# noisystreet/aither

Hardware: AMD Instinct MI355X
Metric: Mcell-updates/sec per iteration (residual+LU-SGS), 256^3 block; % HBM roofline (higher is better)
Workload: dtype f64

## Files before the change

aither_amd/csrc/agx_api.hip:

```cpp
#include "agx_kernels.hpp"
#include "agx_geometry.hpp"
#include "agx_mem.hpp"
#include <rccl/rccl.h>
#include <cstdarg>
#include <cstdio>
#include <cstring>
#include <cstdlib>
#include <cmath>
#include <vector>
#include <array>
#include <map>
#include <string>
#include <algorithm>

using namespace agx;

static char g_err[512] = "";
static int fail(const char* fmt, ...) {
  va_list ap;
  va_start(ap, fmt);
  vsnprintf(g_err, sizeof g_err, fmt, ap);
  va_end(ap);
  return 1;
}
// ... 25 lines not shown
    for (auto& g1 : g) for (auto& g2 : g1) for (auto& g3 : g2)
      if (g3) { hipGraphExecDestroy(g3); g3 = nullptr; }
  }
};

struct Block {
  BlockDev d;
  int global_pos = 0;
  DevBuf<double> slab;
  DevBuf<double> d2;
  DevBuf<double> blockmat;
  DevBuf<double> sweep_rec;
  bool sweep_geo_built = false;
  bool x_planes_current = false;
  bool x_is_zero = false;
  DevBuf<double> mg_forcing, mg_mres, mg_xsave, mg_nodes;
  DevBuf<int> mg_tc, mg_start;
  DevBuf<double> mg_vf, mg_cf;
  const void *mg_tc_key = nullptr, *mg_vf_key = nullptr, *mg_cf_key = nullptr;
  bool node_built = false;
  DevBuf<double> nodes_dev, fcen;
  DevBuf<int> d2_tab;
  std::vector<int> dstart;
  SweepGraphs sweep_graph;
  DevBuf<int> kp_mem;
  unsigned kp_epoch = 0;
  long d2idx(int i, int j, int k) const {
    const int ie = i + d.ng, je = j + d.ng, de = ie + je;
    return (long)(k + d.ng) * d.d2.ps + dstart[de] + je - std::max(0, de - (d.d2.Pi - 1));
  }
// ... 97 lines not shown
  bool halo_batch_required = false;
  int halo_batch_sides = 0;
  long halo_batch_nmax = 0;
  std::vector<int> halo_conn_order;
  struct HaloLevel { int first, sides; long nmax; };
  std::vector<HaloLevel> halo_levels;
  DevBuf<HaloSide> halo_tab_dev[5][2][2];
  bool halo_tab_valid[5][2] = {};
  int halo_set[5] = {};
  PinnedBuf<HaloSide> halo_tab_host;
  int tile_order_inv = TILE_ORDER_STEP;
  int tile_order_visc = TILE_ORDER_STEP;
  std::map<std::array<int, 6>, TilePlan> tile_plans;
  int mresid_split = 1;
  bool mresid_march = true;
  bool have_time_n = false;
  bool have_wall_data = false;
  bool in_iterate = false, ghosts_prefilled = false;
  bool ghost_fill_open = false;
  bool mres_deferred = false;
  hipEvent_t norm_event = nullptr;
  bool consn_pending = false;
  bool state_is_time_n = false;
  long fused_parts = 0;
  bool timing = false;
  std::vector<std::pair<hipEvent_t, hipEvent_t>> ev_pool;
  std::vector<std::pair<int, int>> ev_used;
  double t_ms[G_NGROUP] = {};
  long t_n[G_NGROUP] = {};
};
// ... 84 lines not shown
    HIPCHK(c->stage_buf.alloc(doubles));
  }
  *out = c->stage_buf.get();
  return 0;
}
static int copy_out(agx_ctx* c, double* out, const double* dev, size_t n) {
  HIPCHK(hipGetLastError());
  HIPCHK(hipMemcpyAsync(out, dev, sizeof(double) * n, hipMemcpyDeviceToHost, c->stream));
  HIPCHK(hipStreamSynchronize(c->stream));
  return 0;
}
int upload_aos(agx_ctx* c, Block& b, const double* host, double* const* dst,
               int ncomp, int ci, int cj, int ck, int gsrc) {
  const long n = (long)ci * cj * ck;
  double* tmp = nullptr;
  if (stage_buffer(c, (size_t)n * ncomp, &tmp)) return 1;
  HIPCHK(hipMemcpyAsync(tmp, host, sizeof(double) * n * ncomp,
                        hipMemcpyHostToDevice, c->stream));
  hipLaunchKernelGGL(k_aos_to_soa, dim3((n + 255) / 256), dim3(256), 0,
                     c->stream, tmp, planes(dst, ncomp), ncomp, ci, cj, ck, gsrc, b.d);
  HIPCHK(hipGetLastError());
  HIPCHK(hipStreamSynchronize(c->stream));
  return 0;
}
int download_aos(agx_ctx* c, Block& b, double* host, double* const* src,
                 int ncomp, int ci, int cj, int ck, int gsrc) {
  const long n = (long)ci * cj * ck;
  double* tmp = nullptr;
  if (stage_buffer(c, (size_t)n * ncomp, &tmp)) return 1;
  hipLaunchKernelGGL(k_soa_to_aos, dim3((n + 255) / 256), dim3(256), 0,
// ... 64 lines not shown
      }
}

int ensure_halo_buf(agx_ctx* c, long ndoubles) {
  bool grew;
  HIPCHK(c->halo_buf.reserve((size_t)ndoubles, &grew));
  if (grew)
    for (auto& v : c->halo_tab_valid) v[0] = v[1] = false;
  return 0;
}

int halo_in_d2(const Block& b, int what) { return what == AGX_HALO_UPDATE && b.d.d2.base ? 1 : 0; }
void x_changed(agx_ctx* c) {
  for (auto& blk : c->blocks) blk.x_planes_current = false;
}
Planes5 halo_planes(Block& b, int what) {
  Planes5 r;
  r.rec = what == AGX_HALO_UPDATE ? b.d.sw_dyn : nullptr;
  const bool z2 = halo_in_d2(b, what) != 0;
  r.stride = z2 ? 2 : 1;
#if AGX_NEQ == 7
  if (what == AGX_HALO_TURB) {
    for (int e = 0; e < AGX_NEQ; ++e) r.p[e] = b.d.turb3[e < 3 ? e : 2];
    return r;
  }
#endif
  if (what == AGX_HALO_VELGRAD_A || what == AGX_HALO_VELGRAD_B) {
    for (int e = 0; e < AGX_NEQ; ++e) {
      const int comp = what == AGX_HALO_VELGRAD_A ? e : std::min(5 + e, 8);
      r.p[e] = b.d.vg + (long)comp * b.d.nplane;
// ... 553 lines not shown
  HIPCHK(hipGetLastError());
  return 0;
}

int bc_faces(agx_ctx* c) { Timer t(c, G_BC); return bc_pass(c, true, 0); }
int bc_edges(agx_ctx* c) { Timer t(c, G_BC); return bc_pass(c, false, 0); }

int fill_ghosts(agx_ctx* c) {
  if (bc_faces(c)) return 1;
  if (agx_halo_exchange(c, AGX_HALO_STATE)) return 1;
  return bc_edges(c);
}
int update_pass(agx_ctx* c, int mode, int mm, double* l2, agx_linf* linf) {
  c->state_is_time_n = false;
  const double alpha[4] = {0.25, 1.0 / 3.0, 0.5, 1.0};
  if (mode != 2 && c->fused_pending) {
    Timer t(c, G_UPDATE);
    long off = 0;
    for (size_t n = 0; n < c->blocks.size(); ++n) {
      BlockDev& b = c->blocks[n].d;
      const MarchPlan mp = march_plan(c, b);
      hipLaunchKernelGGL(k_norm_final, dim3(1), dim3(256), 0, c->stream,
                         c->partials.get() + off, mp.nparts, c->norm_out.get() + n);
      off += mp.nparts;
      for (int e = 0; e < AGX_NEQ; ++e) std::swap(b.state[e], b.state2[e]);
    }
    c->halo_set[AGX_HALO_STATE] ^= 1;
    c->fused_pending = false;
    HIPCHK(hipGetLastError());
  } else {
    Timer t(c, G_UPDATE);
    for (size_t n = 0; n < c->blocks.size(); ++n) {
      const BlockDev& b = c->blocks[n].d;
      const int last = mm == c->cfg.nonlinear_iterations - 1;
#if AGX_FAST
      if (mode == 2 && b.d2.base) {
        const dim3 tg((b.ni + TT - 1) / TT, (b.nj + TT - 1) / TT, b.nk);
        hipLaunchKernelGGL(k_update_d2, tg, dim3(256), 0, c->stream, b, c->gas, c->sp, last,
                           c->partials.get());
        if (reduce_norms(c, n, (long)tg.x * tg.y * tg.z)) return 1;
        continue;
      }
#endif
      const dim3 grid = cell_grid(b, CELL_BLOCK);
      hipLaunchKernelGGL(k_update, grid, CELL_BLOCK, 0, c->stream, b, c->gas,
                         c->sp, mode, mode == 1 ? alpha[mm & 3] : 1.0, last,
                         c->partials.get());
      if (reduce_norms(c, n, (long)grid.x * grid.y * grid.z)) return 1;
    }
  }
  HIPCHK(hipMemcpyAsync(c->norm_host.get(), c->norm_out.get(),
                        sizeof(NormPartial) * c->blocks.size(),
                        hipMemcpyDeviceToHost, c->stream));
  if (c->mres_deferred)
    HIPCHK(hipMemcpyAsync(c->norm_host.get() + c->blocks.size(),
                          c->norm_out.get() + c->blocks.size() + 64,
                          sizeof(NormPartial) * c->blocks.size(), hipMemcpyDeviceToHost,
                          c->stream));
  HIPCHK(hipMemcpyAsync(c->err_host.get(), c->err_dev.get(), sizeof(int),
                        hipMemcpyDeviceToHost, c->stream));
  if (c->in_iterate && c->eager_ghosts) {
    if (!c->norm_event) HIPCHK(hipEventCreateWithFlags(&c->norm_event, hipEventDisableTiming));
    HIPCHK(hipEventRecord(c->norm_event, c->stream));
    if (fill_ghosts(c)) return 1;
    c->ghosts_prefilled = true;
    HIPCHK(hipEventSynchronize(c->norm_event));
// ... 393 lines not shown
        return fail("AGX_TILE_ORDER is '%s': step or column", w);
      }
      c->tile_order_inv = c->tile_order_visc = !strcmp(w, "step") ? TILE_ORDER_STEP : TILE_ORDER_COLUMN;
    }
    if (const char* w = getenv("AGX_EAGER_GHOSTS")) c->eager_ghosts = atoi(w) != 0;
    if (const char* w = getenv("AGX_OVERLAP")) c->overlap = atoi(w) != 0;
    if (const char* w = getenv("AGX_LUSGS")) c->lusgs_mode = !strcmp(w, "plane") ? 0 : 1;
    if (const char* w = getenv("AGX_SPIN_LIMIT")) c->spin_limit = std::max(1, atoi(w));
    if (const char* w = getenv("AGX_GRAPHS")) c->use_graphs = atoi(w) != 0;
    if (const char* w = getenv("AGX_SWEEP_ALL")) c->sweep_all_launch = atoi(w) != 0;
    if (const char* w = getenv("AGX_SWEEP_PIPE")) c->sweep_pipe = atoi(w) != 0;
    if (const char* w = getenv("AGX_SWEEP_THREE")) c->sweep_three = atoi(w) != 0;
    if (const char* w = getenv("AGX_SWEEP_RECORDS")) c->sweep_records = atoi(w) != 0;
    if (const char* w = getenv("AGX_MRESID_SPLIT")) c->mresid_split = std::min(64, std::max(1, atoi(w)));
    if (const char* w = getenv("AGX_MRESID")) c->mresid_march = strcmp(w, "plane") != 0;
    if (const char* w = getenv("AGX_HALO_BATCH")) {
      c->halo_batch = strcmp(w, "0") != 0;
      c->halo_batch_required = !strcmp(w, "require");
    }
  }
  HIPCHK(c->err_dev.alloc(1));
  HIPCHK(hipMemset(c->err_dev.get(), 0, sizeof(int)));
  HIPCHK(c->err_host.alloc(1));
  *c->err_host.get() = 0;
  *out = c;
  return 0;
}

void agx_ctx_destroy(agx_ctx* c) {
  if (!c) return;
// ... 541 lines not shown
  }
  return 0;
}
}

int agx_setup_finalize(agx_ctx* c) {
  HIPCHK(hipSetDevice(c->device));
  const int ng = c->cfg.n_ghost;
  if (!c->blocks.empty() && c->blocks[0].node_built && geo_complete(c)) return 1;
  long max_parts = 1, max_halo = 1;
  long march_parts = 0;
  for (auto& blk : c->blocks) {
    const dim3 g = cell_grid(blk.d, CELL_BLOCK);
    max_parts = std::max(max_parts, (long)g.x * g.y * g.z);
    march_parts += march_plan(c, blk.d).nparts;
    if (blk.d.d2.base)
      max_parts = std::max(max_parts, mresid_wgs(c, blk.d));
  }
  max_parts = std::max(max_parts, march_parts);
  for (auto& k : c->conns) {
    const agx_connection& cc = k.c;
    const bool l0 = cc.rank[0] == c->rank, l1 = cc.rank[1] == c->rank;
    if (!l0 && !l1) continue;
    for (int s = 0; s < 2; ++s) {
      const bool mine = s == 0 ? l0 : l1, partner_mine = s == 0 ? l1 : l0;
      if (!mine) continue;
      const int lb = cc.local_block[s];
      if (lb < 0 || lb >= (int)c->blocks.size()) return fail("connection refers to unknown block");
      const Block* partner = partner_mine ? &c->blocks[cc.local_block[1 - s]] : nullptr;
      for (int space = 0; space < (use_d2(c) ? 2 : 1); ++space)
        if (halo_maps(k, s, space, ng, CellIndex{&c->blocks[lb], space},
                      CellIndex{partner, space}, partner_mine, &max_halo))
// ... 26 lines not shown
    if (!seen) per_peer.emplace_back(sl.peer, 1);
    sl.count = r.count;
    sl.send = hb ? r.hsend.get() : r.send.get();
    sl.recv = hb ? r.hrecv.get() : r.recv.get();
    c->slabs.push_back(sl);
    c->remote.push_back(std::move(r));
  }
  if (c->have_ex) {
    const size_t nrec = 1 + (size_t)c->ex.nranks;
    HIPCHK(c->rec_dev.alloc(nrec));
    HIPCHK(c->rec_host.alloc(nrec));
  }
  c->n_partials = max_parts;
  HIPCHK(c->partials.alloc((size_t)max_parts));
  const size_t nb = std::max<size_t>(c->blocks.size(), 1);
  HIPCHK(c->norm_out.alloc(2 * nb + 64));
  HIPCHK(c->norm_host.alloc(2 * nb));
  c->finalized = true;
  return 0;
}

int agx_state_upload(agx_ctx* c, int id, const double* state) {
  c->ghosts_prefilled = false;
  c->state_is_time_n = false;
  if (flush_consn(c)) return 1;
  if (id < 0 || id >= (int)c->blocks.size()) return fail("bad block id %d", id);
  Block& b = c->blocks[id];
  const BlockDev& d = b.d;
  if (upload_aos(c, b, state, d.state, AGX_NEQ, d.ni + 2 * d.ng,
                 d.nj + 2 * d.ng, d.nk + 2 * d.ng, d.ng))
    return 1;
// ... 354 lines not shown
  if (field >= AGX_FIELD_VOLUME && field <= AGX_FIELD_WALL_DIST)
    return fail("field %d (geometry) cannot be uploaded: it is set when the block is created",
                field);
  if (field_info(b, field, &p, &nc, &gh)) return fail("field %d cannot be uploaded", field);
  const int g = gh ? b.d.ng : 0;
  if (upload_aos(c, b, in, p, nc, b.d.ni + 2 * g, b.d.nj + 2 * g, b.d.nk + 2 * g, g)) return 1;
  if (field == AGX_FIELD_UPDATE) b.x_is_zero = false;
  if (field == AGX_FIELD_UPDATE && b.d.d2.base) return d2_x_copy(c, b, 1);
  return 0;
}

static int implicit_begin(agx_ctx* c, int write_x);
int agx_phase_matrix_residual(agx_ctx* c, double* mr);
static int d2_x_copy(agx_ctx* c, Block& b, int to_d2);
#if AGX_FAST
static void d2_prepare(agx_ctx* c, Block& blk, int write_x, int again);
#endif
namespace {
int mg_solver_ok(agx_ctx* c) {
  if (!c->sp.implicit) return fail("multigrid: implicit time integration only");
  return 0;
}
int mg_x_to_planes(agx_ctx* c, Block& b) {
  return b.d.d2.base && !b.x_planes_current ? d2_x_copy(c, b, 0) : 0;
}
int mg_x_from_planes(agx_ctx* c, Block& b) { return b.d.d2.base ? d2_x_copy(c, b, 1) : 0; }
void mg_x_records(agx_ctx* c, Block& b) {
  if (b.d.sw_dyn)
    hipLaunchKernelGGL(k_mg_x_records, dim3((unsigned)((b.d.nplane + 255) / 256)), dim3(256), 0,
                       c->stream, b.d);
}
// ... 64 lines not shown
  return 0;
}
int mg_order(agx_ctx* producer, agx_ctx* consumer) {
  if (producer->stream != consumer->stream) HIPCHK(hipStreamSynchronize(producer->stream));
  return 0;
}
}

int agx_mg_restrict(agx_ctx* f, agx_ctx* cz, int blk, int what, const int32_t* tc,
                    const double* vf) {
  if (mg_check(f, cz, blk)) return 1;
  Block &bf = f->blocks[blk], &bc = cz->blocks[blk];
  if (what < AGX_MG_STATE || what > AGX_MG_FORCING) return fail("mg_restrict: bad selector %d", what);
  if (what != AGX_MG_FORCING && !vf) return fail("mg_restrict: volume weights missing");
  if (flush_consn(f) || flush_consn(cz)) return 1;
  MgMap m;
  if (mg_maps(f, bf, tc, vf, nullptr, bc.d.ni, bc.d.nj, bc.d.nk, &m)) return 1;
  if (what == AGX_MG_UPDATE && mg_x_to_planes(f, bf)) return 1;
  if (what == AGX_MG_FORCING && mg_x_to_planes(cz, bc)) return 1;
  if (mg_order(f, cz)) return 1;
  if (what == AGX_MG_STATE) {
    for (int e = 0; e < AGX_NEQ; ++e)
      HIPCHK(hipMemsetAsync(bc.d.state[e], 0, sizeof(double) * bc.d.nplane, cz->stream));
    cz->ghosts_prefilled = false;
    cz->state_is_time_n = false;
    cz->mg_coarse = true;
  } else if (what == AGX_MG_UPDATE) {
    for (int e = 0; e < AGX_NEQ; ++e)
      HIPCHK(hipMemsetAsync(bc.d.x[e], 0, sizeof(double) * bc.d.nplane, cz->stream));
  } else {
    if (!bf.d.mg_mres) return fail("mg_restrict: the fine level has no matrix residual yet");
    if (mg_planes(cz, bc, bc.mg_forcing, &bc.d.mg_forcing)) return 1;
  }
  hipLaunchKernelGGL(k_mg_restrict, cell_grid(bc.d, CELL_BLOCK), CELL_BLOCK, 0, cz->stream, bf.d,
                     bc.d, m, what);
  if (what == AGX_MG_FORCING)
    hipLaunchKernelGGL(k_mg_axmb, cell_grid(bc.d, CELL_BLOCK), CELL_BLOCK, 0, cz->stream, bc.d,
                       cz->gas, cz->sp);
  if (what == AGX_MG_UPDATE) {
    mg_x_records(cz, bc);
    if (mg_x_from_planes(cz, bc)) return 1;
  }
#if AGX_FAST
  if (what == AGX_MG_FORCING && bc.d.d2.base) d2_prepare(cz, bc, 0, 1);
#endif
  HIPCHK(hipGetLastError());
  return 0;
}

int agx_mg_matrix_residual(agx_ctx* c, double* mr) {
  if (mg_solver_ok(c)) return 1;
  for (auto& blk : c->blocks) {
    if (mg_planes(c, blk, blk.mg_mres, &blk.d.mg_mres)) return 1;
    if (mg_x_to_planes(c, blk)) return 1;
  }
  c->mres_plane_form = true;
  const int rc = agx_phase_matrix_residual(c, mr);
  c->mres_plane_form = false;
  return rc;
// ... 68 lines not shown
}

int agx_phase_bc_faces(agx_ctx* c) {
  if (bc_faces(c)) return 1;
  c->ghost_fill_open = true;
  return 0;
}
int agx_phase_bc_edges(agx_ctx* c) { return bc_edges(c); }

int agx_phase_residual(agx_ctx* c, int mm, double cfl) {
  if (c->cfg.dt_nondim <= 0.0 && cfl <= 0.0)
    return fail("Neither dt or cfl was specified!");
  c->ghost_fill_open = false;
  c->sp.diag_add = c->mg_coarse ? 1 : 0;
  const bool fuse = can_fuse(c);
  const int store_consn = !c->use_gather && all_tile_ok(c) && c->consn_pending && mm == 0;
  if (store_consn) c->consn_pending = false;
  else if (flush_consn(c)) return 1;
  {
    Timer t(c, G_RESID);
    long off = 0;
    for (auto& blk : c->blocks) {
      const MarchPlan mp = march_plan(c, blk.d);
      MarchArgs ma;
      memset(&ma, 0, sizeof ma);
      ma.kchunk = mp.kchunk;
      ma.mode = c->cfg.time_integration == AGX_TIME_RK4 ? 1 : 0;
      ma.store_consn = store_consn;
      const double rk_alpha[4] = {0.25, 1.0 / 3.0, 0.5, 1.0};
      ma.alpha = rk_alpha[mm & 3];
// ... 101 lines not shown
      Timer t(c, G_BC);
      hipLaunchKernelGGL(k_nr_grads, dim3((blk.nr_max + 255) / 256, blk.d.nsurf), dim3(256), 0,
                         c->stream, blk.d, c->gas);
      HIPCHK(hipGetLastError());
    }
  return 0;
}

int agx_phase_explicit_update(agx_ctx* c, int mm, double* l2, agx_linf* linf) {
  const int mode = c->cfg.time_integration == AGX_TIME_RK4 ? 1 : 0;
  return update_pass(c, mode, mm, l2, linf);
}

static int implicit_begin(agx_ctx* c, int write_x);
#if AGX_FAST
static void d2_prepare(agx_ctx* c, Block& blk, int write_x, int again) {
  const BlockDev& b = blk.d;
  const dim3 grid((b.d2.Pi + TT - 1) / TT, (b.d2.Pj + TT - 1) / TT, b.nk + 2 * b.ng);
  hipLaunchKernelGGL(k_lusgs_prepare, grid, dim3(256), 0, c->stream, b, c->gas, c->sp,
                     write_x, write_x ? (unsigned)(++blk.kp_epoch) & 3u : 0u, again);
}
#endif
int agx_phase_implicit_begin(agx_ctx* c) { return implicit_begin(c, 1); }
static int implicit_begin(agx_ctx* c, int write_x) {
  x_changed(c);
  Timer t(c, G_PREPARE);
  c->sp.un_is_u = c->state_is_time_n ? 1 : 0;
  for (auto& blk : c->blocks) {
    const BlockDev& b = blk.d;
#if AGX_FAST
    if (b.d2.base) {
      bool conn = false;
      for (int q = 0; q < 6; ++q) conn = conn || b.side_conn[q] != 0;
      const int wx = write_x && (c->sp.requires_init || conn) ? 1 : 0;
      d2_prepare(c, blk, wx, 0);
      blk.x_is_zero = write_x && !wx;
      continue;
    }
#endif
    if (!c->sp.requires_init && write_x)
      hipLaunchKernelGGL(k_zero5, dim3((b.nplane + 255) / 256), dim3(256), 0,
                         c->stream, planes(b.x), b.nplane);
    hipLaunchKernelGGL(k_implicit_begin, cell_grid(b, CELL_BLOCK), CELL_BLOCK, 0,
                       c->stream, b, c->gas, c->sp, c->err_dev.get(), write_x);
    if (b.sw_geo) {
      hipLaunchKernelGGL(k_sweep_records, dim3((unsigned)((b.nplane + 255) / 256)), dim3(256), 0,
                         c->stream, b, c->sp, blk.sweep_geo_built ? 0 : 1);
      blk.sweep_geo_built = true;
    }
  }
// ... 451 lines not shown
```

aither_amd/csrc/agx_kernels.hpp:

```cpp
#pragma once
#include "agx_device.hpp"
#include "agx_lusgs.hpp"
#include "agx_tile_plan.hpp"

namespace agx {

struct BlockDev {
  int ni, nj, nk, ng;
  int ioff;
  long sx, sxy, nplane;
  int parent;
  double* state[AGX_NEQ];
  double* state2[AGX_NEQ];
  double* fa[3][4];
  double* vol;
  double* cen[3];
  double* wid[3];
  double* resid[AGX_NEQ];
  double* specrad;
  double* dt;
  double* consn[AGX_NEQ];
  double* consnm1[AGX_NEQ];
  double* x[AGX_NEQ];
  double* xold[AGX_NEQ];
// ... 2034 lines not shown
}
__global__ void k_halo_scatter_all(const HaloSide* __restrict__ tab) {
  halo_scatter_side(tab[blockIdx.y], (long)blockIdx.x * blockDim.x + threadIdx.x);
}
__global__ void k_halo_gather(Planes5 a, const long* __restrict__ src, long n,
                              double* __restrict__ buf) {
  halo_gather_side(HaloSide{a, src, n, buf}, (long)blockIdx.x * blockDim.x + threadIdx.x);
}
__global__ void k_halo_scatter(Planes5 a, const long* __restrict__ dst, long n,
                               const double* __restrict__ buf) {
  halo_scatter_side(HaloSide{a, dst, n, const_cast<double*>(buf)},
                    (long)blockIdx.x * blockDim.x + threadIdx.x);
}


__device__ __forceinline__ void norm_block_fold(double* v, double vmax, long long lin,
                                                NormPartial* out) {
  __shared__ double sh[AGX_NEQ + 1][16];
  __shared__ long long shl[16];
  for (int off = 32; off > 0; off >>= 1) {
#pragma unroll
    for (int e = 0; e < AGX_NEQ; ++e) v[e] += __shfl_down(v[e], off, 64);
    const double ov = __shfl_down(vmax, off, 64);
    const long long ol = __shfl_down(lin, off, 64);
    if (ov > vmax || (ov == vmax && ol < lin)) { vmax = ov; lin = ol; }
  }
  const int tid = threadIdx.y * blockDim.x + threadIdx.x;
  const int wave = tid >> 6, lane = tid & 63;
  if (lane == 0) {
#pragma unroll
    for (int e = 0; e < AGX_NEQ; ++e) sh[e][wave] = v[e];
    sh[AGX_NEQ][wave] = vmax;
    shl[wave] = lin;
  }
// ... 4 lines not shown
#pragma unroll
    for (int e = 0; e < AGX_NEQ; ++e) {
      double s = 0.0;
      for (int w = 0; w < nw; ++w) s += sh[e][w];
      p.l2[e] = s;
    }
    p.vmax = sh[AGX_NEQ][0];
    p.lin = shl[0];
    for (int w = 1; w < nw; ++w)
      if (sh[AGX_NEQ][w] > p.vmax || (sh[AGX_NEQ][w] == p.vmax && shl[w] < p.lin)) {
        p.vmax = sh[AGX_NEQ][w];
        p.lin = shl[w];
      }
    *out = p;
  }
}
__device__ __forceinline__ void norm_block_reduce(const double* r, long lin0,
                                                  bool active,
                                                  NormPartial* out) {
  double v[AGX_NEQ];
  double vmax = -1.0e300;
  long long lin = 0x7fffffffffffffffLL;
#pragma unroll
  for (int e = 0; e < AGX_NEQ; ++e) {
    v[e] = active ? r[e] * r[e] : 0.0;
    if (active && r[e] > vmax) { vmax = r[e]; lin = lin0 + e; }
  }
  norm_block_fold(v, vmax, lin, out);
}

// ... 68 lines not shown

__global__ void __launch_bounds__(256)
k_store_time_n(BlockDev b, GasDev g, int also_nm1) {
  const int i = blockIdx.x * blockDim.x + threadIdx.x;
  const int j = blockIdx.y * blockDim.y + threadIdx.y;
  const int k = blockIdx.z;
  if (i >= b.ni || j >= b.nj) return;
  const long q = b.idx(i, j, k);
  double s[AGX_NEQ], u[AGX_NEQ];
  load5(b.state, q, s);
  prim_to_cons(g, s, u);
  store5(b.consn, q, u);
  if (also_nm1) store5(b.consnm1, q, u);
}

__device__ __forceinline__ void rhs_b(const BlockDev& b, const GasDev& g,
                                      const SolverDev& sp, long q, double* out) {
  double r[AGX_NEQ];
  load5(b.resid, q, r);
  const double thetaInv = 1.0 / sp.theta;
  if (sp.un_is_u && !sp.bdf2) {
#pragma unroll
    for (int e = 0; e < AGX_NEQ; ++e) out[e] = -thetaInv * r[e] - 0.0;
    return;
  }
  double s[AGX_NEQ], u[AGX_NEQ], un[AGX_NEQ];
  load5(b.state, q, s);
  load5(b.consn, q, un);
  prim_to_cons(g, s, u);
  const double vdt = b.vol[q] / (b.dt[q] * sp.theta);
  const double cN = vdt * (1.0 + sp.zeta);
#pragma unroll
  for (int e = 0; e < AGX_NEQ; ++e)
    out[e] = -thetaInv * r[e] - (sp.un_is_u ? 0.0 : cN * (u[e] - un[e]));
  if (sp.bdf2) {
    double um[AGX_NEQ];
    load5(b.consnm1, q, um);
    const double cM = vdt * sp.zeta;
#pragma unroll
    for (int e = 0; e < AGX_NEQ; ++e) out[e] += cM * (un[e] - um[e]);
  }
}

__device__ __forceinline__ void rhs_bf(const BlockDev& b, const GasDev& g,
                                       const SolverDev& sp, long q, double* out) {
  rhs_b(b, g, sp, q, out);
  if (b.mg_forcing) {
#pragma unroll
    for (int e = 0; e < AGX_NEQ; ++e) out[e] += b.mg_forcing[(long)e * b.nplane + q];
  }
}

__device__ __forceinline__ void add_off_diag(const BlockDev& b, const GasDev& g,
                                             const SolverDev& sp,
                                             double* const* x, int i, int j,
                                             int k, long q, bool lower,
                                             double sign, double* acc) {
  const int c[3] = {i, j, k};
  const int nn[3] = {b.ni, b.nj, b.nk};
#pragma unroll
  for (int d = 0; d < 3; ++d) {
    const long s = b.stride(d);
    bool use;
    long qn, qf;
    if (lower) {
// ... 1418 lines not shown
```

aither_amd/csrc/agx_lusgs_kernels.hpp:

```cpp
#pragma once

namespace agx {

constexpr int TT = 32;
constexpr int TRS = TT + 2;
__device__ __forceinline__ int tile_diag_index(int li, int lj) {
  const int dd = li + lj;
  if (dd < TT) return dd * (dd + 1) / 2 + lj;
  const int r = 2 * TT - 2 - dd;
  return TT * TT - (r + 1) * (r + 2) / 2 + (lj - (dd - (TT - 1)));
}
__device__ __forceinline__ void tile_table(unsigned short* s_tab) {
  const int tid = threadIdx.x;
#pragma unroll
  for (int m = 0; m < 4; ++m) {
    const int li = tid & (TT - 1), lj = (tid >> 5) + 8 * m;
    s_tab[tile_diag_index(li, lj)] = (unsigned short)(li | (lj << 8));
  }
}

__device__ __forceinline__ double kp_tagged(double v, unsigned tag) {
  const unsigned long long u = (unsigned long long)__double_as_longlong(v);
  return __longlong_as_double((long long)((u & ~3ull) | tag));
}
// ... 36 lines not shown
  const long t = (long)blockIdx.x * blockDim.x + threadIdx.x;
  const long n = (long)z.Pi * z.Pj * (b.nk + 2 * b.ng);
  if (t >= n) return;
  const int ie = (int)(t % z.Pi), je = (int)((t / z.Pi) % z.Pj),
            ke = (int)(t / ((long)z.Pi * z.Pj));
  const long q = b.idx(ie - b.ng, je - b.ng, ke - b.ng);
  const long p = (long)ke * z.ps + z.pos2(ie, je);
#pragma unroll
  for (int e = 0; e < AGX_NEQ; ++e) {
    double* xp = reinterpret_cast<double*>(z.pa(PA_X + (e >> 1))) + 2 * p + (e & 1);
    if (to_d2) *xp = kp_tagged(b.x[e][q], tag);
    else b.x[e][q] = *xp;
  }
}

__global__ void __launch_bounds__(256)
k_lusgs_prepare(BlockDev b, GasDev g, SolverDev sp, int write_x, unsigned tag, int again) {
  __shared__ double sv[6][TT][TRS];
  __shared__ unsigned short s_tab[TT * TT];
  const D2Dev& z = b.d2;
  const int tid = threadIdx.x;
  tile_table(s_tab);
  const int i0 = blockIdx.x * TT, j0 = blockIdx.y * TT, ke = blockIdx.z;
  const int k = ke - b.ng;
  const int li = tid & (TT - 1);
  double bb[4][AGX_NEQ], x0[4][AGX_NEQ], ainv[4], vf[4];
#pragma unroll
  for (int m = 0; m < 4; ++m) {
    const int lj = (tid >> 5) + 8 * m;
    const int ie = i0 + li, je = j0 + lj;
    const int i = ie - b.ng, j = je - b.ng;
#pragma unroll
    for (int e = 0; e < AGX_NEQ; ++e) { bb[m][e] = 0.0; x0[m][e] = 0.0; }
    ainv[m] = 1.0;
    vf[m] = 0.0;
    double cs = 0.0;
    if (ie < z.Pi && je < z.Pj) {
      const long q = b.idx(i, j, k);
      double s[AGX_NEQ];
#pragma unroll
      for (int e = 0; e < AGX_NEQ; ++e) { s[e] = b.state[e][q]; sv[e][lj][li] = s[e]; }
      if (s[0] > 0.0) cs = sound_speed(g, s);
      if (sp.viscous) vf[m] = cell_visc_factor(g, s);
      const bool phys = i >= 0 && i < b.ni && j >= 0 && j < b.nj && k >= 0 && k < b.nk;
      if (phys) {
        double dvt = (b.vol[q] * (1.0 + sp.zeta)) / (b.dt[q] * sp.theta);
        if (sp.dual_time_cfl > 0.0) dvt += fmax(b.specrad[q], 0.0) / sp.dual_time_cfl;
        const double a = again ? b.ainv[q] : b.a[q] * sp.relax + dvt;
        b.ainv[q] = a;
        if (sp.diag_add) b.a[q] = a;
        ainv[m] = 1.0 / a;
        rhs_bf(b, g, sp, q, bb[m]);
        if (sp.requires_init) {
#pragma unroll
          for (int e = 0; e < AGX_NEQ; ++e) x0[m][e] = bb[m][e] * ainv[m];
        }
      }
    }
    sv[5][lj][li] = cs;
  }
  __syncthreads();
  long pos[4];
  int tli[4], tlj[4];
#pragma unroll
  for (int m = 0; m < 4; ++m) {
    const unsigned tl = s_tab[tid + 256 * m];
    tli[m] = tl & 0xff; tlj[m] = tl >> 8;
    const int ie = i0 + tli[m], je = j0 + tlj[m];
    pos[m] = -1;
    if (ie < z.Pi && je < z.Pj) {
      pos[m] = (long)ke * z.ps + z.pos2(ie, je);
#pragma unroll
      for (int h = 0; h < 3; ++h)
        z.pa(PA_S + h)[pos[m]] = make_double2(sv[2 * h][tlj[m]][tli[m]], sv[2 * h + 1][tlj[m]][tli[m]]);
    }
  }
  __syncthreads();
#pragma unroll
  for (int m = 0; m < 4; ++m) {
    const int lj = (tid >> 5) + 8 * m;
#pragma unroll
    for (int e = 0; e < AGX_NEQ; ++e) sv[e][lj][li] = bb[m][e];
    sv[5][lj][li] = ainv[m];
  }
  __syncthreads();
  double ai2[4];
#pragma unroll
  for (int m = 0; m < 4; ++m) {
    ai2[m] = sv[5][tlj[m]][tli[m]];
    if (pos[m] >= 0) {
#pragma unroll
      for (int h = 0; h < 3; ++h)
        z.pa(PA_B + h)[pos[m]] = make_double2(sv[2 * h][tlj[m]][tli[m]], sv[2 * h + 1][tlj[m]][tli[m]]);
    }
  }
  __syncthreads();
#pragma unroll
  for (int m = 0; m < 4; ++m) {
    const int lj = (tid >> 5) + 8 * m;
#pragma unroll
    for (int e = 0; e < AGX_NEQ; ++e) sv[e][lj][li] = x0[m][e];
    sv[5][lj][li] = vf[m];
  }
  __syncthreads();
#pragma unroll
  for (int m = 0; m < 4; ++m) {
    if (pos[m] >= 0) {
      if (write_x) {
        z.pa(PA_X + 0)[pos[m]] = make_double2(kp_tagged(sv[0][tlj[m]][tli[m]], tag),
                                              kp_tagged(sv[1][tlj[m]][tli[m]], tag));
        z.pa(PA_X + 1)[pos[m]] = make_double2(kp_tagged(sv[2][tlj[m]][tli[m]], tag),
                                              kp_tagged(sv[3][tlj[m]][tli[m]], tag));
        z.pa(PA_X + 2)[pos[m]] = make_double2(kp_tagged(sv[4][tlj[m]][tli[m]], tag), ai2[m]);
      }
      if (sp.viscous) z.vf()[pos[m]] = sv[5][tlj[m]][tli[m]];
    }
  }
}

struct KpRec {
  double dx[AGX_NEQ];
  double r1, v1[3], p1, h1;
  double r0, v0[3], p0, h0;
  double cs, vf;
};
constexpr int KP_NV = 19;
template <class G>
__device__ __forceinline__ void kp_build_rec(const G& g, const double* s, double cs,
                                             double vf, const double* dx, KpRec& r) {
  const double ke = g.hf + 0.5 * dot3(s + 1, s + 1);
  const double e0 = s[0] * ke + g.n * s[4];
// ... 466 lines not shown
      }
      if (k < b.nk - 1 || bc_is_connection(b, i, j, k + 1, 6)) col_term(cp, fk1, false, acc);
      const double a = 1.0 / b2.y;
      const double bv[AGX_NEQ] = {b0.x, b0.y, b1.x, b1.y, b2.x};
#pragma unroll
      for (int e = 0; e < AGX_NEQ; ++e) {
        const double r = -(c0.x[e] * a - acc[e] - bv[e]);
        l2[e] += r * r;
      }
      cm = c0; c0 = cp; fk0 = fk1;
    }
  }
  norm_block_fold(l2, -1.0e300, 0x7fffffffffffffffLL, partials + blockIdx.x);
}

__global__ void __launch_bounds__(256)
k_update_d2(BlockDev b, GasDev g, SolverDev sp, int last_mm, NormPartial* partials) {
  __shared__ double sv[AGX_NEQ][TT][TRS];
  __shared__ unsigned short s_tab[TT * TT];
  const D2Dev& z = b.d2;
  const int tid = threadIdx.x;
  tile_table(s_tab);
  __syncthreads();
  const int i0 = blockIdx.x * TT, j0 = blockIdx.y * TT, k = blockIdx.z;
#pragma unroll
  for (int m = 0; m < 4; ++m) {
    const unsigned tl = s_tab[tid + 256 * m];
    const int tli = tl & 0xff, tlj = tl >> 8;
    const int i = i0 + tli, j = j0 + tlj;
    if (i < b.ni && j < b.nj) {
      const long p = (long)(k + b.ng) * z.ps + z.pos2(i + b.ng, j + b.ng);
      const double2 x0 = z.pa(PA_X)[p], x1 = z.pa(PA_X + 1)[p], x2 = z.pa(PA_X + 2)[p];
      sv[0][tlj][tli] = x0.x; sv[1][tlj][tli] = x0.y; sv[2][tlj][tli] = x1.x;
      sv[3][tlj][tli] = x1.y; sv[4][tlj][tli] = x2.x;
    }
  }
  __syncthreads();
  const int li = tid & (TT - 1);
  double l2[AGX_NEQ] = {0, 0, 0, 0, 0};
  double vmax = -1.0e300;
  long long vlin = 0x7fffffffffffffffLL;
#pragma unroll
  for (int m = 0; m < 4; ++m) {
    const int lj = (tid >> 5) + 8 * m;
    const int i = i0 + li, j = j0 + lj;
    if (i < b.ni && j < b.nj) {
      const long q = b.idx(i, j, k);
      double r[AGX_NEQ], s[AGX_NEQ], du[AGX_NEQ], ns[AGX_NEQ];
      load5(b.resid, q, r);
      load5(b.state, q, s);
#pragma unroll
      for (int e = 0; e < AGX_NEQ; ++e) du[e] = sv[e][lj][li];
      update_prim_with_cons(g, s, du, ns);
      store5(b.state, q, ns);
      if (sp.bdf2 && last_mm) {
        double u[AGX_NEQ];
        load5(b.consn, q, u);
        store5(b.consnm1, q, u);
      }
      const long lin0 = (((long)k * b.nj + j) * b.ni + i) * AGX_NEQ;
#pragma unroll
      for (int e = 0; e < AGX_NEQ; ++e) {
        l2[e] += r[e] * r[e];
        if (r[e] > vmax || (r[e] == vmax && lin0 + e < vlin)) { vmax = r[e]; vlin = lin0 + e; }
      }
    }
  }
  const long bid = ((long)blockIdx.z * gridDim.y + blockIdx.y) * gridDim.x + blockIdx.x;
  norm_block_fold(l2, vmax, vlin, partials + bid);
}

}
```

Before: 1478.

## Write d2 state planes in update and move residual norms into prepare

The d2 update kernel now also writes the packed state planes, sound speed and viscous factor for physical cells. This lets the next LU-SGS prepare run in a lean mode that skips re-reading state and recomputing those quantities except on connection ghosts. Residual norms are computed in the prepare kernel, which already loads the residual, so the update kernel can skip its residual read, and cached partials are copied into the norm output. The change adds template variants, staleness flags that must be invalidated on every state or residual write, and an extra norm slot region, which raises the risk of stale-data bugs.

```diff
diff --git a/aither_amd/csrc/agx_api.hip b/aither_amd/csrc/agx_api.hip
--- a/aither_amd/csrc/agx_api.hip
+++ b/aither_amd/csrc/agx_api.hip
@@ -63,6 +63,8 @@
   bool sweep_geo_built = false;
   bool x_planes_current = false;
   bool x_is_zero = false;
+  bool d2_state_current = false;
+  bool resid_norms_current = false;
   DevBuf<double> mg_forcing, mg_mres, mg_xsave, mg_nodes;
   DevBuf<int> mg_tc, mg_start;
   DevBuf<double> mg_vf, mg_cf;
@@ -190,6 +192,8 @@
   std::map<std::array<int, 6>, TilePlan> tile_plans;
   int mresid_split = 1;
   bool mresid_march = true;
+  bool d2_state_update = true;
+  bool resid_norms_prepare = true;
   bool have_time_n = false;
   bool have_wall_data = false;
   bool in_iterate = false, ghosts_prefilled = false;
@@ -304,6 +308,8 @@
                int ncomp, int ci, int cj, int ck, int gsrc) {
   const long n = (long)ci * cj * ck;
   double* tmp = nullptr;
+  b.d2_state_current = false;
+  b.resid_norms_current = false;
   if (stage_buffer(c, (size_t)n * ncomp, &tmp)) return 1;
   HIPCHK(hipMemcpyAsync(tmp, host, sizeof(double) * n * ncomp,
                         hipMemcpyHostToDevice, c->stream));
@@ -398,6 +404,12 @@
 void x_changed(agx_ctx* c) {
   for (auto& blk : c->blocks) blk.x_planes_current = false;
 }
+void state_written(agx_ctx* c) {
+  for (auto& blk : c->blocks) blk.d2_state_current = false;
+}
+void resid_written(agx_ctx* c) {
+  for (auto& blk : c->blocks) blk.resid_norms_current = false;
+}
 Planes5 halo_planes(Block& b, int what) {
   Planes5 r;
   r.rec = what == AGX_HALO_UPDATE ? b.d.sw_dyn : nullptr;
@@ -981,8 +993,11 @@
 int update_pass(agx_ctx* c, int mode, int mm, double* l2, agx_linf* linf) {
   c->state_is_time_n = false;
   const double alpha[4] = {0.25, 1.0 / 3.0, 0.5, 1.0};
+  const size_t nb = c->blocks.size();
+  std::vector<size_t> from_prepare;
   if (mode != 2 && c->fused_pending) {
     Timer t(c, G_UPDATE);
+    state_written(c);
     long off = 0;
     for (size_t n = 0; n < c->blocks.size(); ++n) {
       BlockDev& b = c->blocks[n].d;
@@ -998,17 +1013,32 @@
   } else {
     Timer t(c, G_UPDATE);
     for (size_t n = 0; n < c->blocks.size(); ++n) {
-      const BlockDev& b = c->blocks[n].d;
+      Block& blk = c->blocks[n];
+      const BlockDev& b = blk.d;
       const int last = mm == c->cfg.nonlinear_iterations - 1;
 #if AGX_FAST
       if (mode == 2 && b.d2.base) {
         const dim3 tg((b.ni + TT - 1) / TT, (b.nj + TT - 1) / TT, b.nk);
-        hipLaunchKernelGGL(k_update_d2, tg, dim3(256), 0, c->stream, b, c->gas, c->sp, last,
-                           c->partials.get());
-        if (reduce_norms(c, n, (long)tg.x * tg.y * tg.z)) return 1;
+        const bool ws = c->d2_state_update, pn = blk.resid_norms_current;
+#define AGX_UPD_D2(W, N)                                                                  \
+  hipLaunchKernelGGL((k_update_d2<W, N>), tg, dim3(256), 0, c->stream, b, c->gas, c->sp, \
+                     last, c->partials.get())
+        if (ws && pn) AGX_UPD_D2(1, 0);
+        else if (ws) AGX_UPD_D2(1, 1);
+        else if (pn) AGX_UPD_D2(0, 0);
+        else AGX_UPD_D2(0, 1);
+#undef AGX_UPD_D2
+        blk.d2_state_current = ws;
+        if (pn) {
+          blk.resid_norms_current = false;
+          from_prepare.push_back(n);
+        } else if (reduce_norms(c, n, (long)tg.x * tg.y * tg.z)) {
+          return 1;
+        }
         continue;
       }
 #endif
+      blk.d2_state_current = false;
       const dim3 grid = cell_grid(b, CELL_BLOCK);
       hipLaunchKernelGGL(k_update, grid, CELL_BLOCK, 0, c->stream, b, c->gas,
                          c->sp, mode, mode == 1 ? alpha[mm & 3] : 1.0, last,
@@ -1016,7 +1046,13 @@
       if (reduce_norms(c, n, (long)grid.x * grid.y * grid.z)) return 1;
     }
   }
-  HIPCHK(hipMemcpyAsync(c->norm_host.get(), c->norm_out.get(),
+  const NormPartial* norm_src = c->norm_out.get();
+  if (from_prepare.size() == nb && nb > 0) norm_src += 2 * nb + 64;
+  else
+    for (size_t n : from_prepare)
+      HIPCHK(hipMemcpyAsync(c->norm_out.get() + n, c->norm_out.get() + 2 * nb + 64 + n,
+                            sizeof(NormPartial), hipMemcpyDeviceToDevice, c->stream));
+  HIPCHK(hipMemcpyAsync(c->norm_host.get(), norm_src,
                         sizeof(NormPartial) * c->blocks.size(),
                         hipMemcpyDeviceToHost, c->stream));
   if (c->mres_deferred)
@@ -1440,6 +1476,20 @@
     if (const char* w = getenv("AGX_SWEEP_RECORDS")) c->sweep_records = atoi(w) != 0;
     if (const char* w = getenv("AGX_MRESID_SPLIT")) c->mresid_split = std::min(64, std::max(1, atoi(w)));
     if (const char* w = getenv("AGX_MRESID")) c->mresid_march = strcmp(w, "plane") != 0;
+    if (const char* w = getenv("AGX_D2_STATE")) {
+      if (strcmp(w, "update") && strcmp(w, "prepare")) {
+        delete c;
+        return fail("AGX_D2_STATE is '%s': update or prepare", w);
+      }
+      c->d2_state_update = !strcmp(w, "update");
+    }
+    if (const char* w = getenv("AGX_RESID_NORMS")) {
+      if (strcmp(w, "prepare") && strcmp(w, "update")) {
+        delete c;
+        return fail("AGX_RESID_NORMS is '%s': prepare or update", w);
+      }
+      c->resid_norms_prepare = !strcmp(w, "prepare");
+    }
     if (const char* w = getenv("AGX_HALO_BATCH")) {
       c->halo_batch = strcmp(w, "0") != 0;
       c->halo_batch_required = !strcmp(w, "require");
@@ -2011,8 +2061,13 @@
     const dim3 g = cell_grid(blk.d, CELL_BLOCK);
     max_parts = std::max(max_parts, (long)g.x * g.y * g.z);
     march_parts += march_plan(c, blk.d).nparts;
-    if (blk.d.d2.base)
+    if (blk.d.d2.base) {
       max_parts = std::max(max_parts, mresid_wgs(c, blk.d));
+#if AGX_FAST
+      max_parts = std::max(max_parts, (long)((blk.d.d2.Pi + TT - 1) / TT) *
+                                          ((blk.d.d2.Pj + TT - 1) / TT) * (blk.d.nk + 2 * blk.d.ng));
+#endif
+    }
   }
   max_parts = std::max(max_parts, march_parts);
   for (auto& k : c->conns) {
@@ -2069,7 +2124,7 @@
   c->n_partials = max_parts;
   HIPCHK(c->partials.alloc((size_t)max_parts));
   const size_t nb = std::max<size_t>(c->blocks.size(), 1);
-  HIPCHK(c->norm_out.alloc(2 * nb + 64));
+  HIPCHK(c->norm_out.alloc(3 * nb + 64));
   HIPCHK(c->norm_host.alloc(2 * nb));
   c->finalized = true;
   return 0;
@@ -2454,7 +2509,7 @@
 int agx_phase_matrix_residual(agx_ctx* c, double* mr);
 static int d2_x_copy(agx_ctx* c, Block& b, int to_d2);
 #if AGX_FAST
-static void d2_prepare(agx_ctx* c, Block& blk, int write_x, int again);
+static int d2_prepare(agx_ctx* c, Block& blk, int write_x, int again, int norms);
 #endif
 namespace {
 int mg_solver_ok(agx_ctx* c) {
@@ -2549,6 +2604,8 @@
   if (what < AGX_MG_STATE || what > AGX_MG_FORCING) return fail("mg_restrict: bad selector %d", what);
   if (what != AGX_MG_FORCING && !vf) return fail("mg_restrict: volume weights missing");
   if (flush_consn(f) || flush_consn(cz)) return 1;
+  bc.d2_state_current = false;
+  bc.resid_norms_current = false;
   MgMap m;
   if (mg_maps(f, bf, tc, vf, nullptr, bc.d.ni, bc.d.nj, bc.d.nk, &m)) return 1;
   if (what == AGX_MG_UPDATE && mg_x_to_planes(f, bf)) return 1;
@@ -2577,7 +2634,7 @@
     if (mg_x_from_planes(cz, bc)) return 1;
   }
 #if AGX_FAST
-  if (what == AGX_MG_FORCING && bc.d.d2.base) d2_prepare(cz, bc, 0, 1);
+  if (what == AGX_MG_FORCING && bc.d.d2.base && d2_prepare(cz, bc, 0, 1, 0)) return 1;
 #endif
   HIPCHK(hipGetLastError());
   return 0;
@@ -2676,6 +2733,8 @@
   c->ghost_fill_open = false;
   c->sp.diag_add = c->mg_coarse ? 1 : 0;
   const bool fuse = can_fuse(c);
+  resid_written(c);
+  if (fuse) state_written(c);
   const int store_consn = !c->use_gather && all_tile_ok(c) && c->consn_pending && mm == 0;
   if (store_consn) c->consn_pending = false;
   else if (flush_consn(c)) return 1;
@@ -2807,11 +2866,28 @@
 
 static int implicit_begin(agx_ctx* c, int write_x);
 #if AGX_FAST
-static void d2_prepare(agx_ctx* c, Block& blk, int write_x, int again) {
+static int d2_prepare(agx_ctx* c, Block& blk, int write_x, int again, int norms) {
   const BlockDev& b = blk.d;
   const dim3 grid((b.d2.Pi + TT - 1) / TT, (b.d2.Pj + TT - 1) / TT, b.nk + 2 * b.ng);
-  hipLaunchKernelGGL(k_lusgs_prepare, grid, dim3(256), 0, c->stream, b, c->gas, c->sp,
-                     write_x, write_x ? (unsigned)(++blk.kp_epoch) & 3u : 0u, again);
+  const bool lean = blk.d2_state_current && !again;
+  int ghost_s = 0;
+  for (int q = 0; q < 6; ++q) ghost_s |= b.side_conn[q] != 0;
+  const unsigned tag = write_x ? (unsigned)(++blk.kp_epoch) & 3u : 0u;
+#define AGX_PREP(L, N)                                                                       \
+  hipLaunchKernelGGL((k_lusgs_prepare<L, N>), grid, dim3(256), 0, c->stream, b, c->gas, c->sp, \
+                     write_x, tag, again, ghost_s, c->partials.get())
+  if (lean && norms) AGX_PREP(1, 1);
+  else if (lean) AGX_PREP(1, 0);
+  else if (norms) AGX_PREP(0, 1);
+  else AGX_PREP(0, 0);
+#undef AGX_PREP
+  if (norms) {
+    const size_t n = (size_t)(&blk - c->blocks.data()), nb = c->blocks.size();
+    if (reduce_norms(c, n, (long)grid.x * grid.y * grid.z, c->norm_out.get() + 2 * nb + 64 + n))
+      return 1;
+    blk.resid_norms_current = true;
+  }
+  return 0;
 }
 #endif
 int agx_phase_implicit_begin(agx_ctx* c) { return implicit_begin(c, 1); }
@@ -2826,7 +2902,7 @@
       bool conn = false;
       for (int q = 0; q < 6; ++q) conn = conn || b.side_conn[q] != 0;
       const int wx = write_x && (c->sp.requires_init || conn) ? 1 : 0;
-      d2_prepare(c, blk, wx, 0);
+      if (d2_prepare(c, blk, wx, 0, write_x && c->resid_norms_prepare ? 1 : 0)) return 1;
       blk.x_is_zero = write_x && !wx;
       continue;
     }
diff --git a/aither_amd/csrc/agx_kernels.hpp b/aither_amd/csrc/agx_kernels.hpp
--- a/aither_amd/csrc/agx_kernels.hpp
+++ b/aither_amd/csrc/agx_kernels.hpp
@@ -2072,10 +2072,9 @@
 }
 
 
-__device__ __forceinline__ void norm_block_fold(double* v, double vmax, long long lin,
-                                                NormPartial* out) {
-  __shared__ double sh[AGX_NEQ + 1][16];
-  __shared__ long long shl[16];
+__device__ __forceinline__ void norm_block_fold_in(double* v, double vmax, long long lin,
+                                                   NormPartial* out, double (*sh)[16],
+                                                   long long* shl) {
   for (int off = 32; off > 0; off >>= 1) {
 #pragma unroll
     for (int e = 0; e < AGX_NEQ; ++e) v[e] += __shfl_down(v[e], off, 64);
@@ -2110,6 +2109,12 @@
       }
     *out = p;
   }
+}
+__device__ __forceinline__ void norm_block_fold(double* v, double vmax, long long lin,
+                                                NormPartial* out) {
+  __shared__ double sh[AGX_NEQ + 1][16];
+  __shared__ long long shl[16];
+  norm_block_fold_in(v, vmax, lin, out, sh, shl);
 }
 __device__ __forceinline__ void norm_block_reduce(const double* r, long lin0,
                                                   bool active,
@@ -2208,10 +2213,9 @@
   if (also_nm1) store5(b.consnm1, q, u);
 }
 
-__device__ __forceinline__ void rhs_b(const BlockDev& b, const GasDev& g,
-                                      const SolverDev& sp, long q, double* out) {
-  double r[AGX_NEQ];
-  load5(b.resid, q, r);
+__device__ __forceinline__ void rhs_b_r(const BlockDev& b, const GasDev& g,
+                                        const SolverDev& sp, long q, const double* r,
+                                        double* out) {
   const double thetaInv = 1.0 / sp.theta;
   if (sp.un_is_u && !sp.bdf2) {
 #pragma unroll
@@ -2235,14 +2239,27 @@
     for (int e = 0; e < AGX_NEQ; ++e) out[e] += cM * (un[e] - um[e]);
   }
 }
-
+__device__ __forceinline__ void rhs_b(const BlockDev& b, const GasDev& g,
+                                      const SolverDev& sp, long q, double* out) {
+  double r[AGX_NEQ];
+  load5(b.resid, q, r);
+  rhs_b_r(b, g, sp, q, r, out);
+}
+
+__device__ __forceinline__ void rhs_bf_r(const BlockDev& b, const GasDev& g,
+                                         const SolverDev& sp, long q, const double* r,
+                                         double* out) {
+  rhs_b_r(b, g, sp, q, r, out);
+  if (b.mg_forcing) {
+#pragma unroll
+    for (int e = 0; e < AGX_NEQ; ++e) out[e] += b.mg_forcing[(long)e * b.nplane + q];
+  }
+}
 __device__ __forceinline__ void rhs_bf(const BlockDev& b, const GasDev& g,
                                        const SolverDev& sp, long q, double* out) {
-  rhs_b(b, g, sp, q, out);
-  if (b.mg_forcing) {
-#pragma unroll
-    for (int e = 0; e < AGX_NEQ; ++e) out[e] += b.mg_forcing[(long)e * b.nplane + q];
-  }
+  double r[AGX_NEQ];
+  load5(b.resid, q, r);
+  rhs_bf_r(b, g, sp, q, r, out);
 }
 
 __device__ __forceinline__ void add_off_diag(const BlockDev& b, const GasDev& g,
diff --git a/aither_amd/csrc/agx_lusgs_kernels.hpp b/aither_amd/csrc/agx_lusgs_kernels.hpp
--- a/aither_amd/csrc/agx_lusgs_kernels.hpp
+++ b/aither_amd/csrc/agx_lusgs_kernels.hpp
@@ -74,8 +74,10 @@
   }
 }
 
+template <int LEAN, int NORMS>
 __global__ void __launch_bounds__(256)
-k_lusgs_prepare(BlockDev b, GasDev g, SolverDev sp, int write_x, unsigned tag, int again) {
+k_lusgs_prepare(BlockDev b, GasDev g, SolverDev sp, int write_x, unsigned tag, int again,
+                int ghost_s, NormPartial* partials) {
   __shared__ double sv[6][TT][TRS];
   __shared__ unsigned short s_tab[TT * TT];
   const D2Dev& z = b.d2;
@@ -85,6 +87,9 @@
   const int k = ke - b.ng;
   const int li = tid & (TT - 1);
   double bb[4][AGX_NEQ], x0[4][AGX_NEQ], ainv[4], vf[4];
+  double l2[AGX_NEQ] = {0, 0, 0, 0, 0};
+  double vmax = -1.0e300;
+  long long vlin = 0x7fffffffffffffffLL;
 #pragma unroll
   for (int m = 0; m < 4; ++m) {
     const int lj = (tid >> 5) + 8 * m;
@@ -97,12 +102,14 @@
     double cs = 0.0;
     if (ie < z.Pi && je < z.Pj) {
       const long q = b.idx(i, j, k);
-      double s[AGX_NEQ];
-#pragma unroll
-      for (int e = 0; e < AGX_NEQ; ++e) { s[e] = b.state[e][q]; sv[e][lj][li] = s[e]; }
-      if (s[0] > 0.0) cs = sound_speed(g, s);
-      if (sp.viscous) vf[m] = cell_visc_factor(g, s);
       const bool phys = i >= 0 && i < b.ni && j >= 0 && j < b.nj && k >= 0 && k < b.nk;
+      if (!LEAN || (ghost_s && !phys)) {
+        double s[AGX_NEQ];
+#pragma unroll
+        for (int e = 0; e < AGX_NEQ; ++e) { s[e] = b.state[e][q]; sv[e][lj][li] = s[e]; }
+        if (s[0] > 0.0) cs = sound_speed(g, s);
+        if (sp.viscous) vf[m] = cell_visc_factor(g, s);
+      }
       if (phys) {
         double dvt = (b.vol[q] * (1.0 + sp.zeta)) / (b.dt[q] * sp.theta);
         if (sp.dual_time_cfl > 0.0) dvt += fmax(b.specrad[q], 0.0) / sp.dual_time_cfl;
@@ -110,7 +117,17 @@
         b.ainv[q] = a;
         if (sp.diag_add) b.a[q] = a;
         ainv[m] = 1.0 / a;
-        rhs_bf(b, g, sp, q, bb[m]);
+        double r[AGX_NEQ];
+        load5(b.resid, q, r);
+        rhs_bf_r(b, g, sp, q, r, bb[m]);
+        if (NORMS) {
+          const long lin0 = (((long)k * b.nj + j) * b.ni + i) * AGX_NEQ;
+#pragma unroll
+          for (int e = 0; e < AGX_NEQ; ++e) {
+            l2[e] += r[e] * r[e];
+            if (r[e] > vmax || (r[e] == vmax && lin0 + e < vlin)) { vmax = r[e]; vlin = lin0 + e; }
+          }
+        }
         if (sp.requires_init) {
 #pragma unroll
           for (int e = 0; e < AGX_NEQ; ++e) x0[m][e] = bb[m][e] * ainv[m];
@@ -122,17 +139,25 @@
   __syncthreads();
   long pos[4];
   int tli[4], tlj[4];
+  bool st_s[4];
 #pragma unroll
   for (int m = 0; m < 4; ++m) {
     const unsigned tl = s_tab[tid + 256 * m];
     tli[m] = tl & 0xff; tlj[m] = tl >> 8;
     const int ie = i0 + tli[m], je = j0 + tlj[m];
     pos[m] = -1;
+    st_s[m] = !LEAN;
     if (ie < z.Pi && je < z.Pj) {
       pos[m] = (long)ke * z.ps + z.pos2(ie, je);
-#pragma unroll
-      for (int h = 0; h < 3; ++h)
-        z.pa(PA_S + h)[pos[m]] = make_double2(sv[2 * h][tlj[m]][tli[m]], sv[2 * h + 1][tlj[m]][tli[m]]);
+      if (LEAN) {
+        const int i = ie - b.ng, j = je - b.ng;
+        st_s[m] = ghost_s && !(i >= 0 && i < b.ni && j >= 0 && j < b.nj && k >= 0 && k < b.nk);
+      }
+      if (st_s[m]) {
+#pragma unroll
+        for (int h = 0; h < 3; ++h)
+          z.pa(PA_S + h)[pos[m]] = make_double2(sv[2 * h][tlj[m]][tli[m]], sv[2 * h + 1][tlj[m]][tli[m]]);
+      }
     }
   }
   __syncthreads();
@@ -154,27 +179,36 @@
         z.pa(PA_B + h)[pos[m]] = make_double2(sv[2 * h][tlj[m]][tli[m]], sv[2 * h + 1][tlj[m]][tli[m]]);
     }
   }
-  __syncthreads();
-#pragma unroll
-  for (int m = 0; m < 4; ++m) {
-    const int lj = (tid >> 5) + 8 * m;
-#pragma unroll
-    for (int e = 0; e < AGX_NEQ; ++e) sv[e][lj][li] = x0[m][e];
-    sv[5][lj][li] = vf[m];
-  }
-  __syncthreads();
-#pragma unroll
-  for (int m = 0; m < 4; ++m) {
-    if (pos[m] >= 0) {
-      if (write_x) {
-        z.pa(PA_X + 0)[pos[m]] = make_double2(kp_tagged(sv[0][tlj[m]][tli[m]], tag),
-                                              kp_tagged(sv[1][tlj[m]][tli[m]], tag));
-        z.pa(PA_X + 1)[pos[m]] = make_double2(kp_tagged(sv[2][tlj[m]][tli[m]], tag),
-                                              kp_tagged(sv[3][tlj[m]][tli[m]], tag));
-        z.pa(PA_X + 2)[pos[m]] = make_double2(kp_tagged(sv[4][tlj[m]][tli[m]], tag), ai2[m]);
-      }
-      if (sp.viscous) z.vf()[pos[m]] = sv[5][tlj[m]][tli[m]];
-    }
+  if (!LEAN || write_x || ghost_s) {
+    __syncthreads();
+#pragma unroll
+    for (int m = 0; m < 4; ++m) {
+      const int lj = (tid >> 5) + 8 * m;
+#pragma unroll
+      for (int e = 0; e < AGX_NEQ; ++e) sv[e][lj][li] = x0[m][e];
+      sv[5][lj][li] = vf[m];
+    }
+    __syncthreads();
+#pragma unroll
+    for (int m = 0; m < 4; ++m) {
+      if (pos[m] >= 0) {
+        if (write_x) {
+          z.pa(PA_X + 0)[pos[m]] = make_double2(kp_tagged(sv[0][tlj[m]][tli[m]], tag),
+                                                kp_tagged(sv[1][tlj[m]][tli[m]], tag));
+          z.pa(PA_X + 1)[pos[m]] = make_double2(kp_tagged(sv[2][tlj[m]][tli[m]], tag),
+                                                kp_tagged(sv[3][tlj[m]][tli[m]], tag));
+          z.pa(PA_X + 2)[pos[m]] = make_double2(kp_tagged(sv[4][tlj[m]][tli[m]], tag), ai2[m]);
+        }
+        if (sp.viscous && st_s[m]) z.vf()[pos[m]] = sv[5][tlj[m]][tli[m]];
+      }
+    }
+  }
+  if (NORMS) {
+    __syncthreads();
+    const long bid = ((long)blockIdx.z * gridDim.y + blockIdx.y) * gridDim.x + blockIdx.x;
+    norm_block_fold_in(l2, vmax, vlin, partials + bid,
+                       reinterpret_cast<double(*)[16]>(&sv[0][0][0]),
+                       reinterpret_cast<long long*>(&sv[1][0][0]));
   }
 }
 
@@ -671,6 +705,7 @@
   norm_block_fold(l2, -1.0e300, 0x7fffffffffffffffLL, partials + blockIdx.x);
 }
 
+template <int WRITE_S, int NORMS>
 __global__ void __launch_bounds__(256)
 k_update_d2(BlockDev b, GasDev g, SolverDev sp, int last_mm, NormPartial* partials) {
   __shared__ double sv[AGX_NEQ][TT][TRS];
@@ -680,16 +715,20 @@
   tile_table(s_tab);
   __syncthreads();
   const int i0 = blockIdx.x * TT, j0 = blockIdx.y * TT, k = blockIdx.z;
+  long pos[4];
+  int tli[4], tlj[4];
 #pragma unroll
   for (int m = 0; m < 4; ++m) {
     const unsigned tl = s_tab[tid + 256 * m];
-    const int tli = tl & 0xff, tlj = tl >> 8;
-    const int i = i0 + tli, j = j0 + tlj;
+    tli[m] = tl & 0xff; tlj[m] = tl >> 8;
+    const int i = i0 + tli[m], j = j0 + tlj[m];
+    pos[m] = -1;
     if (i < b.ni && j < b.nj) {
       const long p = (long)(k + b.ng) * z.ps + z.pos2(i + b.ng, j + b.ng);
+      pos[m] = p;
       const double2 x0 = z.pa(PA_X)[p], x1 = z.pa(PA_X + 1)[p], x2 = z.pa(PA_X + 2)[p];
-      sv[0][tlj][tli] = x0.x; sv[1][tlj][tli] = x0.y; sv[2][tlj][tli] = x1.x;
-      sv[3][tlj][tli] = x1.y; sv[4][tlj][tli] = x2.x;
+      sv[0][tlj[m]][tli[m]] = x0.x; sv[1][tlj[m]][tli[m]] = x0.y; sv[2][tlj[m]][tli[m]] = x1.x;
+      sv[3][tlj[m]][tli[m]] = x1.y; sv[4][tlj[m]][tli[m]] = x2.x;
     }
   }
   __syncthreads();
@@ -697,34 +736,85 @@
   double l2[AGX_NEQ] = {0, 0, 0, 0, 0};
   double vmax = -1.0e300;
   long long vlin = 0x7fffffffffffffffLL;
+  double nsk[4][AGX_NEQ], cs[4], vf[4];
 #pragma unroll
   for (int m = 0; m < 4; ++m) {
     const int lj = (tid >> 5) + 8 * m;
     const int i = i0 + li, j = j0 + lj;
+    cs[m] = 0.0;
+    vf[m] = 0.0;
+    if (WRITE_S) {
+#pragma unroll
+      for (int e = 0; e < AGX_NEQ; ++e) nsk[m][e] = 0.0;
+    }
     if (i < b.ni && j < b.nj) {
       const long q = b.idx(i, j, k);
       double r[AGX_NEQ], s[AGX_NEQ], du[AGX_NEQ], ns[AGX_NEQ];
-      load5(b.resid, q, r);
+      if (NORMS) load5(b.resid, q, r);
       load5(b.state, q, s);
 #pragma unroll
       for (int e = 0; e < AGX_NEQ; ++e) du[e] = sv[e][lj][li];
       update_prim_with_cons(g, s, du, ns);
       store5(b.state, q, ns);
+      if (WRITE_S) {
+#pragma unroll
+        for (int e = 0; e < AGX_NEQ; ++e) nsk[m][e] = ns[e];
+        if (ns[0] > 0.0) cs[m] = sound_speed(g, ns);
+        if (sp.viscous) vf[m] = cell_visc_factor(g, ns);
+      }
       if (sp.bdf2 && last_mm) {
         double u[AGX_NEQ];
         load5(b.consn, q, u);
         store5(b.consnm1, q, u);
       }
-      const long lin0 = (((long)k * b.nj + j) * b.ni + i) * AGX_NEQ;
-#pragma unroll
-      for (int e = 0; e < AGX_NEQ; ++e) {
-        l2[e] += r[e] * r[e];
-        if (r[e] > vmax || (r[e] == vmax && lin0 + e < vlin)) { vmax = r[e]; vlin = lin0 + e; }
-      }
-    }
-  }
-  const long bid = ((long)blockIdx.z * gridDim.y + blockIdx.y) * gridDim.x + blockIdx.x;
-  norm_block_fold(l2, vmax, vlin, partials + bid);
-}
-
-}
+      if (NORMS) {
+        const long lin0 = (((long)k * b.nj + j) * b.ni + i) * AGX_NEQ;
+#pragma unroll
+        for (int e = 0; e < AGX_NEQ; ++e) {
+          l2[e] += r[e] * r[e];
+          if (r[e] > vmax || (r[e] == vmax && lin0 + e < vlin)) { vmax = r[e]; vlin = lin0 + e; }
+        }
+      }
+    }
+  }
+  if (WRITE_S) {
+    __syncthreads();
+#pragma unroll
+    for (int m = 0; m < 4; ++m) {
+      const int lj = (tid >> 5) + 8 * m;
+#pragma unroll
+      for (int e = 0; e < AGX_NEQ; ++e) sv[e][lj][li] = nsk[m][e];
+    }
+    __syncthreads();
+    double pp[4];
+#pragma unroll
+    for (int m = 0; m < 4; ++m) {
+      pp[m] = sv[4][tlj[m]][tli[m]];
+      if (pos[m] >= 0) {
+        z.pa(PA_S + 0)[pos[m]] = make_double2(sv[0][tlj[m]][tli[m]], sv[1][tlj[m]][tli[m]]);
+        z.pa(PA_S + 1)[pos[m]] = make_double2(sv[2][tlj[m]][tli[m]], sv[3][tlj[m]][tli[m]]);
+      }
+    }
+    __syncthreads();
+#pragma unroll
+    for (int m = 0; m < 4; ++m) {
+      const int lj = (tid >> 5) + 8 * m;
+      sv[0][lj][li] = cs[m];
+      sv[1][lj][li] = vf[m];
+    }
+    __syncthreads();
+#pragma unroll
+    for (int m = 0; m < 4; ++m) {
+      if (pos[m] >= 0) {
+        z.pa(PA_S + 2)[pos[m]] = make_double2(pp[m], sv[0][tlj[m]][tli[m]]);
+        if (sp.viscous) z.vf()[pos[m]] = sv[1][tlj[m]][tli[m]];
+      }
+    }
+  }
+  if (NORMS) {
+    const long bid = ((long)blockIdx.z * gridDim.y + blockIdx.y) * gridDim.x + blockIdx.x;
+    norm_block_fold(l2, vmax, vlin, partials + bid);
+  }
+}
+
+}
```

New measurement: 1509, median of 6. +2.1%, better.
